# rrahn/libspm

Measured on AMD Instinct MI355X. Metric: Gbases/s scanned, Myers k<=3 |P|=100, higher is better.
Workload: dtype u32

## Files before the change

### libspm_amd/csrc/filter.hpp

```cpp
#pragma once

#include "brute.hpp"
#include "common.hpp"
#include "filter_shared.hpp"
#include "pack.hpp"
#include "hd.hpp"

namespace spm_hip
{

struct survivor
{
    uint32_t key;
    uint32_t t_lo, t_hi;
    uint32_t pad;
};
constexpr uint32_t kSurvInvalid = 0xFFFFFFFFu;

struct band_rec
{
    uint32_t slot;
    uint32_t val;
    uint32_t seg;
    uint32_t band;
// ... 46 lines not shown
        atomicAdd(counter, (unsigned long long)v);
}

__device__ __forceinline__ uint32_t *cand_chunk_of(const filter_params &P, const uint32_t *lds)
{
    const uint32_t wave = (uint32_t)__builtin_amdgcn_readfirstlane(threadIdx.x >> 6);
    return const_cast<uint32_t *>(lds) + P.lds_words + kCandLdsSlot + kCandRec * wave;
}

__device__ __forceinline__ void span_open(const filter_params &P, const uint32_t *lds, uint32_t lane, uint64_t begin)
{
    if (lane == 0) {
        uint32_t *ck = cand_chunk_of(P, lds);
        ck[4] = 0;
        ck[5] = 0;
        ck[6] = (uint32_t)begin;
        ck[7] = (uint32_t)(begin >> 32);
    }
}

__device__ __forceinline__ void span_give_up(const filter_params &P, uint32_t *ck, uint32_t lane)
{
    if (lane == 0) {
        ck[5] = 1;
        const unsigned long long i = atomicAdd(&P.counters[6], 1ull);
        if (i < P.ovf_cap) {
            P.ovf_spans[2 * i] = ((uint64_t)ck[7] << 32) | ck[6];
            P.ovf_spans[2 * i + 1] = (uint64_t)P.span_chunks * (uint64_t)P.span_unit;
        } else {
            atomicAdd(&P.counters[2], 1ull);
        }
    }
    __builtin_amdgcn_fence(__ATOMIC_RELEASE, "wavefront");
    __builtin_amdgcn_wave_barrier();
}

__device__ __forceinline__ void surv_close(const filter_params &P, const uint32_t *ck, uint32_t lane)
{
    const uint32_t used = ck[2], size = ck[3];
    const uint64_t base = ((uint64_t)ck[1] << 32) | ck[0];
    for (uint32_t i = used + lane; i < size; i += 64)
        if (base + i < P.surv_cap) {
            survivor sv;
            sv.key = 0;
            sv.t_lo = 0;
            sv.t_hi = kSurvInvalid;
            sv.pad = 0;
            P.surv[base + i] = sv;
        }
}

__device__ __forceinline__ void emit_survivors(const filter_params &P, bool has, uint32_t key, uint64_t t, uint32_t lane,
                                               const uint32_t *lds)
{
    const uint64_t m = __ballot(has);
    if (m == 0)
        return;
    uint32_t *ck = cand_chunk_of(P, lds);
    const uint32_t n = __popcll(m);
    uint32_t used = (uint32_t)__builtin_amdgcn_readfirstlane(ck[2]);
    const uint32_t size = (uint32_t)__builtin_amdgcn_readfirstlane(ck[3]);
    const uint32_t cnt = (uint32_t)__builtin_amdgcn_readfirstlane(ck[4]) + n;
    if (cnt > P.span_budget) {
        span_give_up(P, ck, lane);
        return;
    }
    if (used + n > size) {
        surv_close(P, ck, lane);
        uint32_t next = size * 2 < kChunkMin ? kChunkMin : (size * 2 > kChunkMax ? kChunkMax : size * 2);
        next = next < n ? n : next;
        if (lane == 0) {
            const unsigned long long b = atomicAdd(&P.counters[1], (unsigned long long)next);
            ck[0] = (uint32_t)b;
            ck[1] = (uint32_t)(b >> 32);
            ck[2] = 0;
            ck[3] = next;
        }
        used = 0;
        __builtin_amdgcn_fence(__ATOMIC_RELEASE, "wavefront");
        __builtin_amdgcn_wave_barrier();
    }
    const uint64_t cbase = ((uint64_t)(uint32_t)__builtin_amdgcn_readfirstlane(ck[1]) << 32) |
                           (uint32_t)__builtin_amdgcn_readfirstlane(ck[0]);
    if (cbase + used + n > P.surv_cap) {
        span_give_up(P, ck, lane);
        return;
    }
    if (has) {
        survivor sv;
        sv.key = key;
        sv.t_lo = (uint32_t)t;
        sv.t_hi = (uint32_t)(t >> 32);
        sv.pad = P.pass;
        P.surv[cbase + used + __popcll(m & ((1ull << lane) - 1))] = sv;
    }
    if (lane == 0) {
        ck[2] = used + n;
        ck[4] = cnt;
    }
    __builtin_amdgcn_fence(__ATOMIC_RELEASE, "wavefront");
    __builtin_amdgcn_wave_barrier();
}

template <int S, int NWD, int HV, int SIG, bool PK, bool KM>
__device__ __forceinline__ void filter_words(const filter_params &P, const uint32_t (&w)[NWD],
                                             const uint32_t (&prev)[NWD], const uint32_t (&nv)[SIG != 4 ? NWD : 1],
                                             uint64_t gbase, uint32_t lane, const uint32_t *lds, uint32_t idx_mask)
{
    constexpr int NWIN = 16 / S;
    const uint32_t kmask = KM ? P.key_mask : 0xFFFFFFFFu;
    static_assert(NWD * NWIN <= 32, "one mask bit per window of a group");
    uint32_t pos_mask = 0;
    if constexpr (HV == 2) {
        const uint16_t *fp_tab = reinterpret_cast<const uint16_t *>(lds);
        const uint16_t *disp_tab = reinterpret_cast<const uint16_t *>(reinterpret_cast<const uint8_t *>(lds) + P.chd_disp_off);
        uint32_t xs[NWD * NWIN], ds[NWD * NWIN];
#pragma unroll
        for (int u = 0; u < NWD; ++u) {
#pragma unroll
            for (int i = 0; i < NWIN; ++i) {
                const int d = S * (i + 1);
                const uint32_t key = (d == 16 ? w[u] : alignbit(w[u], prev[u], (2 * d) & 31)) & kmask;
                const uint32_t x = chd_hash(key).x;
                xs[u * NWIN + i] = x;
                ds[u * NWIN + i] = disp_tab[x >> P.chd_bucket_shift];
            }
        }
#pragma unroll
        for (int u = 0; u < NWD; ++u) {
#pragma unroll
            for (int i = 0; i < NWIN; ++i) {
                const int d = S * (i + 1);
                const uint32_t key = (d == 16 ? w[u] : alignbit(w[u], prev[u], (2 * d) & 31)) & kmask;
                const uint32_t slot = ((xs[u * NWIN + i] >> 3) + ds[u * NWIN + i] * ((key | 1u) & 0xFFFFFFu)) &
                                      P.chd_slot_mask;
                ds[u * NWIN + i] = fp_tab[slot];
            }
        }
#pragma unroll
        for (int u = 0; u < NWD; ++u) {
#pragma unroll
            for (int i = 0; i < NWIN; ++i) {
                const int d = S * (i + 1);
                const uint32_t key = (d == 16 ? w[u] : alignbit(w[u], prev[u], (2 * d) & 31)) & kmask;
                const uint32_t miss = (ds[u * NWIN + i] ^ key ^ (key >> 16)) & 0xFFFFu;
                pos_mask |= (miss == 0 ? 1u : 0u) << (u * NWIN + i);
            }
        }
    } else {
#pragma unroll
        for (int u = 0; u < NWD; ++u) {
#pragma unroll
            for (int i = 0; i < NWIN; ++i) {
                const int d = S * (i + 1);
                const uint32_t key = (d == 16 ? w[u] : alignbit(w[u], prev[u], (2 * d) & 31)) & kmask;
                const uint32_t h = bloom_hash(key, 0) & idx_mask;
                const uint32_t word = lds[h >> 5];
                pos_mask |= __builtin_amdgcn_ubfe(word, h, 1) << (u * NWIN + i);
            }
        }
        for (uint32_t pr = 1; pr < P.n_probes; ++pr) {
            if (__ballot(pos_mask != 0) == 0)
                break;
            uint32_t keep = 0;
#pragma unroll
            for (int u = 0; u < NWD; ++u) {
#pragma unroll
                for (int i = 0; i < NWIN; ++i) {
                    if (pos_mask & (1u << (u * NWIN + i))) {
                        const int d = S * (i + 1);
                        const uint32_t key = (d == 16 ? w[u] : alignbit(w[u], prev[u], (2 * d) & 31)) & kmask;
                        const uint32_t h = bloom_hash(key, pr) & idx_mask;
                        const uint32_t word = lds[h >> 5];
                        keep |= __builtin_amdgcn_ubfe(word, h, 1) << (u * NWIN + i);
                    }
                }
            }
            pos_mask = keep;
        }
    }
    if constexpr (SIG != 4) {
        if (__ballot(pos_mask != 0) != 0) {
#pragma unroll
            for (int u = 0; u < NWD; ++u) {
#pragma unroll
                for (int i = 0; i < NWIN; ++i) {
                    const int d = S * (i + 1);
                    if (__builtin_amdgcn_ubfe(nv[u], d, P.key_len) != 0)
                        pos_mask &= ~(1u << (u * NWIN + i));
                }
            }
        }
    }
    while (__ballot(pos_mask != 0) != 0) {
        if (__builtin_amdgcn_readfirstlane(cand_chunk_of(P, lds)[5]) != 0)
            break;
        uint64_t t = 0;
        uint32_t key = 0;
        bool has = false;
        if (pos_mask != 0) {
            const int bit = __ffs(pos_mask) - 1;
            pos_mask &= pos_mask - 1;
            const int u = bit / NWIN, i = bit % NWIN;
            const int d = S * (i + 1);
            uint32_t wu = w[0], pu = prev[0];
#pragma unroll
            for (int q = 1; q < NWD; ++q)
                if (u == q) {
                    wu = w[q];
                    pu = prev[q];
                }
            key = (d == 16 ? wu : alignbit(wu, pu, (uint32_t)(2 * d) & 31u)) & kmask;
            const uint64_t wpos = PK ? gbase + (uint64_t)(u >> 2) * 4096 + (uint64_t)lane * 64 + (uint64_t)(u & 3) * 16
                                     : gbase + (uint64_t)u * 1024 + (uint64_t)lane * 16;
            const int64_t ts = (int64_t)wpos - 16 + d;
            if (ts >= (int64_t)P.lo && (uint64_t)ts + P.key_len <= P.hi) {
                t = (uint64_t)ts;
                has = true;
            }
        }
        emit_survivors(P, has, key, t, lane, lds);
    }
}



__device__ __forceinline__ uint32_t anchor_select(uint32_t w, uint32_t prev, uint32_t c, uint32_t cm)
{
    const uint32_t C0 = (c & 3u) * 0x55555555u, M0 = (cm & 3u) * 0x55555555u;
    const uint32_t C1 = (c >> 2) * 0x55555555u, M1 = (cm >> 2) * 0x55555555u;
    const uint32_t X = alignbit(w, prev, 2);
    const uint32_t Y = alignbit(w, prev, 4);
    uint32_t t = ((X ^ C0) & M0) | ((Y ^ C1) & M1);
    t |= t >> 1;
    return ~t & 0x55555555u;
}

template <int NWD>
__device__ __forceinline__ void filter_words_anchored(const filter_params &P, const uint32_t (&w)[NWD], const uint32_t (&prev)[NWD],
                                                      uint64_t gbase, uint32_t lane, const uint32_t *lds)
{
    static_assert(NWD % 2 == 0 || NWD == 1, "words are taken in pairs");
    const uint16_t *fp_tab = reinterpret_cast<const uint16_t *>(lds);
    const uint16_t *disp_tab = reinterpret_cast<const uint16_t *>(reinterpret_cast<const uint8_t *>(lds) + P.chd_disp_off);
#pragma unroll
    for (int j = 0; j < NWD; j += 2) {
        uint32_t todo = anchor_select(w[j], prev[j], P.anchor_c, P.anchor_cm);
        if (j + 1 < NWD)
            todo |= anchor_select(w[j + 1 < NWD ? j + 1 : j], prev[j + 1 < NWD ? j + 1 : j], P.anchor_c, P.anchor_cm) << 1;
        while (__ballot(todo != 0) != 0) {
            const bool act = todo != 0;
            const uint32_t b = act ? (uint32_t)__ffs(todo) - 1u : 0u;
            todo &= todo - 1;
            const uint32_t u = b & 1u, d = (b >> 1) + 1u;
            const uint32_t wu = (j + 1 < NWD && u) ? w[j + 1 < NWD ? j + 1 : j] : w[j];
            const uint32_t pu = (j + 1 < NWD && u) ? prev[j + 1 < NWD ? j + 1 : j] : prev[j];
            const uint32_t key = (uint32_t)((((uint64_t)wu << 32) | pu) >> (2 * d));
            const uint32_t x = chd_hash(key).x;
            const uint32_t dsp = disp_tab[x >> P.chd_bucket_shift];
            const uint32_t slot = ((x >> 3) + dsp * ((key | 1u) & 0xFFFFFFu)) & P.chd_slot_mask;
            const uint32_t f = fp_tab[slot];
            const bool hit = act && ((f ^ key ^ (key >> 16)) & 0xFFFFu) == 0;
            if (__ballot(hit) != 0) {
                if (__builtin_amdgcn_readfirstlane(cand_chunk_of(P, lds)[5]) != 0)
                    return;
                const uint64_t wpos = gbase + (uint64_t)(j + u) * 1024 + (uint64_t)lane * 16;
                const int64_t ts = (int64_t)wpos - 16 + (int64_t)d;
                const bool has = hit && ts >= (int64_t)P.lo && (uint64_t)ts + P.key_len <= P.hi;
                emit_survivors(P, has, key, has ? (uint64_t)ts : 0, lane, lds);
            }
        }
    }
}

template <int S, int UU, int HV, int SIG, bool KM, bool AN = false>
__device__ __forceinline__ void filter_group(const filter_params &P, const uint4 (&cur)[UU], uint64_t gbase,
                                             uint32_t &carry_in, uint32_t &carry_n, uint32_t lane,
                                             const uint32_t *lds, uint32_t idx_mask)
{
    uint32_t w[UU], prev[UU];
    uint32_t nv[SIG != 4 ? UU : 1];
#pragma unroll
    for (int u = 0; u < UU; ++u) {
        uint32_t nm = 0;
        w[u] = pack16_sig<SIG>(cur[u], nm);
        prev[u] = __builtin_amdgcn_update_dpp(0u, w[u], 0x138 , 0xF, 0xF, false);
        if (lane == 0)
            prev[u] = carry_in;
        carry_in = __builtin_amdgcn_readlane(w[u], 63);
        if (SIG != 4) {
            uint32_t np = __builtin_amdgcn_update_dpp(0u, nm, 0x138, 0xF, 0xF, false);
            if (lane == 0)
                np = carry_n;
            carry_n = __builtin_amdgcn_readlane(nm, 63);
            nv[u] = (nm << 16) | np;
        }
    }
    if constexpr (AN)
        filter_words_anchored<UU>(P, w, prev, gbase, lane, lds);
    else
        filter_words<S, UU, HV, SIG, false, KM>(P, w, prev, nv, gbase, lane, lds, idx_mask);
}

template <int S, int U, int HV, int SIG, bool KM, bool AN = false>
__global__ __launch_bounds__(((S == 1 && !KM && SIG == 4) || (S == 2 && U == 2)) ? 1024 : 512) void seed_filter_kernel(const filter_params P)
{
    extern __shared__ uint32_t lds[];
    for (uint32_t i = threadIdx.x; i < P.lds_words; i += blockDim.x)
        lds[i] = P.bitmap[i];
    if ((threadIdx.x & 63) == 0) {
        uint32_t *ck = lds + P.lds_words + kCandLdsSlot + kCandRec * (threadIdx.x >> 6);
        for (uint32_t i = 0; i < kCandRec; ++i)
            ck[i] = 0;
    }
    __syncthreads();

    const uint32_t lane = threadIdx.x & 63;
    const uint32_t waves_per_wg = blockDim.x >> 6;
    const uint64_t wave_id =
        (uint64_t)blockIdx.x * waves_per_wg + (uint32_t)__builtin_amdgcn_readfirstlane(threadIdx.x >> 6);
    const uint64_t n_waves = (uint64_t)gridDim.x * waves_per_wg;
    const uint32_t idx_mask = P.bitmap_words * 32 - 1;

    const uint64_t base0 = P.lo & ~1023ull;
    const uint64_t n_chunks = (P.hi - base0 + 1023) / 1024;
    const uint64_t n_whole = (P.hi - base0) / 1024;
    const uint64_t span = P.span_chunks;
    const uint64_t n_spans = (n_chunks + span - 1) / span;
    const uint8_t *lane_text = P.text + base0 + (uint64_t)lane * 16;

    const uint32_t wave_in_wg = (uint32_t)__builtin_amdgcn_readfirstlane(threadIdx.x >> 6);
    uint64_t sp = wave_id;
    for (;;) {
        if (P.dynamic == 1) {
            unsigned long long t = 0;
            if (lane == 0)
                t = atomicAdd(&P.counters[4], 1ull);
            sp = ((unsigned long long)__builtin_amdgcn_readfirstlane((uint32_t)(t >> 32)) << 32) |
                 (uint32_t)__builtin_amdgcn_readfirstlane((uint32_t)t);
        } else if (P.dynamic == 2) {
            __syncthreads();
            if (threadIdx.x == 0) {
                const unsigned long long t = atomicAdd(&P.counters[4], (unsigned long long)waves_per_wg);
                lds[P.lds_words] = (uint32_t)t;
                lds[P.lds_words + 1] = (uint32_t)(t >> 32);
            }
            __syncthreads();
            const uint64_t base = ((uint64_t)(uint32_t)__builtin_amdgcn_readfirstlane(lds[P.lds_words + 1]) << 32) |
                                  (uint32_t)__builtin_amdgcn_readfirstlane(lds[P.lds_words]);
            if (base >= n_spans)
                break;
            sp = base + wave_in_wg;
            if (sp >= n_spans)
                continue;
        }
        if (sp >= n_spans)
            break;
        const uint64_t c_begin = sp * span;
        const uint64_t c_end = c_begin + span < n_chunks ? c_begin + span : n_chunks;
        span_open(P, lds, lane, base0 + c_begin * 1024);
        uint32_t carry_in = 0, carry_n = 0;
        {
            const uint64_t cb = base0 + c_begin * 1024;
            if (cb >= 16 && lane == 0) {
                const uint4 before = load_text16(P.text, cb - 16, P.hi);
                carry_in = pack16_sig<SIG>(before, carry_n);
            }
            carry_in = __builtin_amdgcn_readfirstlane(carry_in);
            carry_n = __builtin_amdgcn_readfirstlane(carry_n);
        }
        uint64_t ch = c_begin;
        const uint64_t whole_end = c_end < n_whole ? c_end : n_whole;
        const uint64_t fast_end = c_begin + (whole_end > c_begin ? (whole_end - c_begin) / U * U : 0);
        if (ch < fast_end) {
            uint4 nxt[U];
#pragma unroll
            for (int u = 0; u < U; ++u)
                nxt[u] = load16_stream(lane_text + (ch + u) * 1024);
            for (; ch < fast_end; ch += U) {
                uint4 cur[U];
#pragma unroll
                for (int u = 0; u < U; ++u)
                    cur[u] = nxt[u];
                const bool more = ch + U < fast_end;
                const uint64_t pf = more ? ch + U : ch;
                const uint64_t ustride = more ? 1024 : 0;
#pragma unroll
                for (int u = 0; u < U; ++u)
                    nxt[u] = load16_stream(lane_text + pf * 1024 + (uint64_t)u * ustride);
                if constexpr (S <= 2)
                    __builtin_amdgcn_sched_barrier(0);
                filter_group<S, U, HV, SIG, KM, AN>(P, cur, base0 + ch * 1024, carry_in, carry_n, lane, lds, idx_mask);
            }
        }
        for (; ch < c_end; ++ch) {
            uint4 one[1];
            one[0] = load_text16(P.text, base0 + ch * 1024 + (uint64_t)lane * 16, P.hi);
            filter_group<S, 1, HV, SIG, KM, AN>(P, one, base0 + ch * 1024, carry_in, carry_n, lane, lds, idx_mask);
        }
        sp += n_waves;
    }
    surv_close(P, cand_chunk_of(P, lds), lane);
}

constexpr uint32_t kDenseQueueCap = 192;
constexpr int kDenseBatches = 3;

template <int NP>
__device__ __forceinline__ uint32_t dense_select(const filter_params &P, uint32_t w, uint32_t prev)
{
    const uint32_t X = alignbit(w, prev, 2);
    const uint32_t Y = alignbit(w, prev, 4);
    uint32_t sel = 0;
#pragma unroll
    for (int i = 0; i < NP; ++i) {
        const uint32_t C0 = (P.pat_c[i] & 3u) * 0x55555555u, M0 = (P.pat_cm[i] & 3u) * 0x55555555u;
        const uint32_t C1 = (P.pat_c[i] >> 2) * 0x55555555u, M1 = (P.pat_cm[i] >> 2) * 0x55555555u;
        uint32_t t = ((X ^ C0) & M0) | ((Y ^ C1) & M1);
        t |= t >> 1;
        sel |= ~t;
    }
    return sel & 0x55555555u;
}

struct dense_queue
{
    uint32_t key[kDenseQueueCap];
    uint32_t off[kDenseQueueCap];
};

__device__ __forceinline__ void dense_drain(const filter_params &P, dense_queue &Q, uint32_t &qn, bool all, uint64_t span_base,
                                            uint32_t lane, const uint32_t *lds)
{
    while (qn >= 64 || (all && qn != 0)) {
        const uint32_t nb_full = qn >> 6;
        uint32_t nb = all ? (qn + 63) >> 6 : nb_full;
        nb = nb > (uint32_t)kDenseBatches ? (uint32_t)kDenseBatches : nb;
        uint32_t key[kDenseBatches], off[kDenseBatches];
        uint4 bk[kDenseBatches];
        bool v[kDenseBatches];
#pragma unroll
        for (int b = 0; b < kDenseBatches; ++b) {
            const int32_t e = (int32_t)qn - 64 * b - 1 - (int32_t)lane;
            v[b] = (uint32_t)b < nb && e >= 0;
            key[b] = 0;
            off[b] = 0;
            bk[b] = make_uint4(0, 0, 0, 0);
            if (v[b]) {
                key[b] = Q.key[e];
                off[b] = Q.off[e];
                bk[b] = P.buckets[dense_bucket(key[b], P.bucket_shift)];
            }
        }
        qn = qn > 64 * nb ? qn - 64 * nb : 0;
#pragma unroll
        for (int b = 0; b < kDenseBatches; ++b) {
            if ((uint32_t)b >= nb)
                break;
            const uint32_t f2 = dense_fp(key[b]) * 0x00010001u;
            const uint32_t x0 = bk[b].x ^ f2, x1 = bk[b].y ^ f2, x2 = bk[b].z ^ f2, x3 = bk[b].w ^ f2;
            const uint32_t z = ((x0 - 0x00010001u) & ~x0) | ((x1 - 0x00010001u) & ~x1) | ((x2 - 0x00010001u) & ~x2) |
                               ((x3 - 0x00010001u) & ~x3);
            const bool hit = v[b] && ((z & 0x80008000u) != 0 || (bk[b].w >> 16) == kDenseAcceptAll);
            if (__ballot(hit) != 0) {
                if (__builtin_amdgcn_readfirstlane(cand_chunk_of(P, lds)[5]) == 0) {
                    const int64_t ts = (int64_t)span_base + (int64_t)off[b] - 16;
                    const bool has = hit && ts >= (int64_t)P.lo && (uint64_t)ts + P.key_len <= P.hi;
                    emit_survivors(P, has, key[b], has ? (uint64_t)ts : 0, lane, lds);
                }
            }
        }
    }
}

template <int UU, int NP, int S, bool KM>
__device__ __forceinline__ void dense_group(const filter_params &P, const uint4 (&cur)[UU], uint64_t gbase, uint64_t span_base,
                                            uint32_t &carry_in, uint32_t lane, const uint32_t *lds, dense_queue &Q, uint32_t &qn)
{
    static_assert(UU % 2 == 0 || UU == 1, "words are taken in pairs");
    uint32_t w[UU], prev[UU];
#pragma unroll
    for (int u = 0; u < UU; ++u) {
        w[u] = pack16(cur[u]);
        prev[u] = __builtin_amdgcn_update_dpp(0u, w[u], 0x138 , 0xF, 0xF, false);
        if (lane == 0)
            prev[u] = carry_in;
        carry_in = __builtin_amdgcn_readlane(w[u], 63);
    }
    const uint32_t goff = (uint32_t)(gbase - span_base) + lane * 16;
#pragma unroll
    for (int j = 0; j < UU; j += 2) {
        constexpr bool pair = UU > 1;
        const uint32_t w0 = w[j], p0 = prev[j], w1 = w[pair ? j + 1 : j], p1 = prev[pair ? j + 1 : j];
        const uint32_t kmask = KM ? P.key_mask : 0xFFFFFFFFu;
        static_assert(kDenseBloomBits == 20, "the word address below takes bits 5..19 of the index");
        uint32_t pm = 0;
        if constexpr (S == 0) {
            uint32_t todo = dense_select<NP>(P, w0, p0);
            if (pair)
                todo |= dense_select<NP>(P, w1, p1) << 1;
            while (todo != 0) {
                const uint32_t b = (uint32_t)__ffs(todo) - 1u;
                todo &= todo - 1;
                const bool odd = (b & 1u) != 0;
                const uint64_t both = ((uint64_t)(odd ? w1 : w0) << 32) | (odd ? p1 : p0);
                const uint32_t key = (uint32_t)(both >> ((b & ~1u) + 2u));
                const uint32_t h = key ^ (key >> 13);
                const uint32_t word = *reinterpret_cast<const uint32_t *>(reinterpret_cast<const uint8_t *>(lds) + ((h >> 3) & 0x1FFFCu));
                pm |= __builtin_amdgcn_ubfe(word, h, 1) << b;
            }
        } else {
#pragma unroll
            for (int u = 0; u < (pair ? 2 : 1); ++u) {
#pragma unroll
                for (int d = S; d <= 16; d += S) {
                    const uint32_t wu = u ? w1 : w0, pu = u ? p1 : p0;
                    const uint32_t key = (d == 16 ? wu : alignbit(wu, pu, (2 * d) & 31)) & kmask;
                    const uint32_t h = key ^ (key >> 13);
                    const uint32_t word = *reinterpret_cast<const uint32_t *>(reinterpret_cast<const uint8_t *>(lds) + ((h >> 3) & 0x1FFFCu));
                    pm |= __builtin_amdgcn_ubfe(word, h, 1) << (2 * (d - 1) + u);
                }
            }
        }
        while (__ballot(pm != 0) != 0) {
            const bool pos = pm != 0;
            const uint32_t b = pos ? (uint32_t)__ffs(pm) - 1u : 0u;
            pm &= pm - 1;
            const bool odd = (b & 1u) != 0;
            const uint64_t both = ((uint64_t)(odd ? w1 : w0) << 32) | (odd ? p1 : p0);
            const uint32_t key = (uint32_t)(both >> ((b & ~1u) + 2u)) & kmask;
            const uint64_t mm = __ballot(pos);
            if (pos) {
                const uint32_t q = qn + __popcll(mm & ((1ull << lane) - 1));
                Q.key[q] = key;
                Q.off[q] = goff + (uint32_t)j * 1024u + (odd ? 1024u : 0u) + (b >> 1) + 1u;
            }
            qn += __popcll(mm);
            __builtin_amdgcn_fence(__ATOMIC_RELEASE, "wavefront");
            __builtin_amdgcn_wave_barrier();
            if (qn > kDenseQueueCap - 64)
                dense_drain(P, Q, qn, false, span_base, lane, lds);
        }
    }
}

template <int U, int NP, int S = 0, bool KM = false>
__global__ __launch_bounds__(1024) void seed_filter_dense_kernel(const filter_params P)
{
    extern __shared__ uint32_t lds[];
    for (uint32_t i = threadIdx.x; i < P.lds_words; i += blockDim.x)
        lds[i] = P.bitmap[i];
    if ((threadIdx.x & 63) == 0) {
        uint32_t *ck = lds + P.lds_words + kCandLdsSlot + kCandRec * (threadIdx.x >> 6);
        for (uint32_t i = 0; i < kCandRec; ++i)
            ck[i] = 0;
    }
    __syncthreads();

    const uint32_t lane = threadIdx.x & 63;
    const uint32_t waves_per_wg = blockDim.x >> 6;
    const uint32_t wave_in_wg = (uint32_t)__builtin_amdgcn_readfirstlane(threadIdx.x >> 6);
    const uint64_t wave_id = (uint64_t)blockIdx.x * waves_per_wg + wave_in_wg;
    const uint64_t n_waves = (uint64_t)gridDim.x * waves_per_wg;
    dense_queue &Q = *reinterpret_cast<dense_queue *>(lds + P.lds_words + kCandLdsSlot + kCandRec * 16 +
                                                      (sizeof(dense_queue) / 4) * wave_in_wg);
    uint32_t qn = 0;

    const uint64_t base0 = P.lo & ~1023ull;
    const uint64_t n_chunks = (P.hi - base0 + 1023) / 1024;
    const uint64_t n_whole = (P.hi - base0) / 1024;
    const uint64_t span = P.span_chunks;
    const uint64_t n_spans = (n_chunks + span - 1) / span;
    const uint8_t *lane_text = P.text + base0 + (uint64_t)lane * 16;

    uint64_t sp = wave_id;
    for (;;) {
        if (P.dynamic == 1) {
            unsigned long long t = 0;
            if (lane == 0)
                t = atomicAdd(&P.counters[4], 1ull);
            sp = ((unsigned long long)__builtin_amdgcn_readfirstlane((uint32_t)(t >> 32)) << 32) |
                 (uint32_t)__builtin_amdgcn_readfirstlane((uint32_t)t);
        } else if (P.dynamic == 2) {
            __syncthreads();
            if (threadIdx.x == 0) {
                const unsigned long long t = atomicAdd(&P.counters[4], (unsigned long long)waves_per_wg);
                lds[P.lds_words] = (uint32_t)t;
                lds[P.lds_words + 1] = (uint32_t)(t >> 32);
            }
            __syncthreads();
            const uint64_t base = ((uint64_t)(uint32_t)__builtin_amdgcn_readfirstlane(lds[P.lds_words + 1]) << 32) |
                                  (uint32_t)__builtin_amdgcn_readfirstlane(lds[P.lds_words]);
            if (base >= n_spans)
                break;
            sp = base + wave_in_wg;
            if (sp >= n_spans)
                continue;
        }
        if (sp >= n_spans)
            break;
        const uint64_t c_begin = sp * span;
        const uint64_t c_end = c_begin + span < n_chunks ? c_begin + span : n_chunks;
        const uint64_t span_base = base0 + c_begin * 1024;
        span_open(P, lds, lane, span_base);
        uint32_t carry_in = 0;
        {
            uint32_t nm = 0;
            if (span_base >= 16 && lane == 0)
                carry_in = pack16_sig<4>(load_text16(P.text, span_base - 16, P.hi), nm);
            carry_in = __builtin_amdgcn_readfirstlane(carry_in);
        }
        uint64_t ch = c_begin;
        const uint64_t whole_end = c_end < n_whole ? c_end : n_whole;
        const uint64_t fast_end = c_begin + (whole_end > c_begin ? (whole_end - c_begin) / U * U : 0);
        if (ch < fast_end) {
            uint4 nxt[U];
#pragma unroll
            for (int u = 0; u < U; ++u)
                nxt[u] = load16_stream(lane_text + (ch + u) * 1024);
            for (; ch < fast_end; ch += U) {
                uint4 cur[U];
#pragma unroll
                for (int u = 0; u < U; ++u)
                    cur[u] = nxt[u];
                const bool more = ch + U < fast_end;
                const uint64_t pf = more ? ch + U : ch;
                const uint64_t ustride = more ? 1024 : 0;
#pragma unroll
                for (int u = 0; u < U; ++u)
                    nxt[u] = load16_stream(lane_text + pf * 1024 + (uint64_t)u * ustride);
                __builtin_amdgcn_sched_barrier(0);
                dense_group<U, NP, S, KM>(P, cur, base0 + ch * 1024, span_base, carry_in, lane, lds, Q, qn);
            }
        }
        for (; ch < c_end; ++ch) {
            uint4 one[1];
            one[0] = load_text16(P.text, base0 + ch * 1024 + (uint64_t)lane * 16, P.hi);
            dense_group<1, NP, S, KM>(P, one, base0 + ch * 1024, span_base, carry_in, lane, lds, Q, qn);
        }
        dense_drain(P, Q, qn, true, span_base, lane, lds);
        sp += n_waves;
    }
    surv_close(P, cand_chunk_of(P, lds), lane);
}

template <int S, int U2, int HV, bool KM>
__global__ __launch_bounds__(1024) void seed_filter_packed_kernel(const filter_params P, const uint4 *__restrict__ shadow)
{
    extern __shared__ uint32_t lds[];
    for (uint32_t i = threadIdx.x; i < P.lds_words; i += blockDim.x)
        lds[i] = P.bitmap[i];
    if ((threadIdx.x & 63) == 0) {
        uint32_t *ck = lds + P.lds_words + kCandLdsSlot + kCandRec * (threadIdx.x >> 6);
        for (uint32_t i = 0; i < kCandRec; ++i)
            ck[i] = 0;
    }
    __syncthreads();

    constexpr int NWD = 4 * U2;
    const uint32_t lane = threadIdx.x & 63;
    const uint32_t waves_per_wg = blockDim.x >> 6;
    const uint32_t wave_in_wg = (uint32_t)__builtin_amdgcn_readfirstlane(threadIdx.x >> 6);
    const uint64_t wave_id = (uint64_t)blockIdx.x * waves_per_wg + wave_in_wg;
    const uint64_t n_waves = (uint64_t)gridDim.x * waves_per_wg;
    const uint32_t idx_mask = P.bitmap_words * 32 - 1;

    const uint64_t base0 = P.lo & ~4095ull;
    const uint64_t n_chunks = (P.hi - base0 + 4095) / 4096;
    const uint64_t span = P.span_chunks;
    const uint64_t n_spans = (n_chunks + span - 1) / span;
    const uint4 *lane_src = shadow + (base0 / 64) + lane;

    uint64_t sp = wave_id;
    for (;;) {
        if (P.dynamic == 1) {
            unsigned long long t = 0;
            if (lane == 0)
                t = atomicAdd(&P.counters[4], 1ull);
            sp = ((unsigned long long)__builtin_amdgcn_readfirstlane((uint32_t)(t >> 32)) << 32) |
                 (uint32_t)__builtin_amdgcn_readfirstlane((uint32_t)t);
        } else if (P.dynamic == 2) {
            __syncthreads();
            if (threadIdx.x == 0) {
                const unsigned long long t = atomicAdd(&P.counters[4], (unsigned long long)waves_per_wg);
                lds[P.lds_words] = (uint32_t)t;
                lds[P.lds_words + 1] = (uint32_t)(t >> 32);
            }
            __syncthreads();
            const uint64_t base = ((uint64_t)(uint32_t)__builtin_amdgcn_readfirstlane(lds[P.lds_words + 1]) << 32) |
                                  (uint32_t)__builtin_amdgcn_readfirstlane(lds[P.lds_words]);
            if (base >= n_spans)
                break;
            sp = base + wave_in_wg;
            if (sp >= n_spans)
                continue;
        }
        if (sp >= n_spans)
            break;
        const uint64_t c_begin = sp * span;
        const uint64_t c_end = c_begin + span < n_chunks ? c_begin + span : n_chunks;
        const uint64_t fast_end = c_begin + (c_end - c_begin + U2 - 1) / U2 * U2;
        span_open(P, lds, lane, base0 + c_begin * 4096);
        uint32_t carry_in = 0;
        {
            const uint64_t first_word = (base0 + c_begin * 4096) / 16;
            if (first_word > 0 && lane == 0)
                carry_in = reinterpret_cast<const uint32_t *>(shadow)[first_word - 1];
            carry_in = __builtin_amdgcn_readfirstlane(carry_in);
        }
        uint4 nxt[U2];
#pragma unroll
        for (int u = 0; u < U2; ++u)
            nxt[u] = load16_stream(reinterpret_cast<const uint8_t *>(lane_src + (c_begin + u) * 64));
        for (uint64_t ch = c_begin; ch < fast_end; ch += U2) {
            uint4 cur[U2];
#pragma unroll
            for (int u = 0; u < U2; ++u)
                cur[u] = nxt[u];
            const bool more = ch + U2 < fast_end;
            const uint64_t pf = more ? ch + U2 : ch;
            const uint64_t ustride = more ? 64 : 0;
#pragma unroll
            for (int u = 0; u < U2; ++u)
                nxt[u] = load16_stream(reinterpret_cast<const uint8_t *>(lane_src + pf * 64 + (uint64_t)u * ustride));
            __builtin_amdgcn_sched_barrier(0);
            uint32_t w[NWD], prev[NWD];
            const uint32_t nv[1] = {0};
#pragma unroll
            for (int u = 0; u < U2; ++u) {
                w[4 * u + 0] = cur[u].x;
                w[4 * u + 1] = cur[u].y;
                w[4 * u + 2] = cur[u].z;
                w[4 * u + 3] = cur[u].w;
                uint32_t p0 = __builtin_amdgcn_update_dpp(0u, cur[u].w, 0x138 , 0xF, 0xF, false);
                if (lane == 0)
                    p0 = carry_in;
                carry_in = __builtin_amdgcn_readlane(cur[u].w, 63);
                prev[4 * u + 0] = p0;
                prev[4 * u + 1] = cur[u].x;
                prev[4 * u + 2] = cur[u].y;
                prev[4 * u + 3] = cur[u].z;
            }
            filter_words<S, NWD, HV, 4, true, KM>(P, w, prev, nv, base0 + ch * 4096, lane, lds, idx_mask);
        }
        sp += n_waves;
    }
    surv_close(P, cand_chunk_of(P, lds), lane);
}

struct verify_params
{
    const uint8_t *text;
    uint64_t text_alloc;
    uint64_t ctx_begin;
    uint64_t scan_begin;
    uint64_t scan_end;
    uint64_t pos_offset;
    const band_rec *bands;
    const unsigned long long *counters;
    uint32_t band_counter;
    uint32_t preselected;
    uint64_t band_cap;
    ulonglong2 *band_tab;
    uint32_t table_mask, band_bits;
    uint32_t runs;
    const uint8_t *surplus;
    uint32_t Bw;
    uint32_t overlap;
    uint32_t max_m;
    const uint32_t *peq32;
    uint32_t sigma;
    uint32_t nw_table;
    uint32_t max_k;
    const int32_t *m;
    const int32_t *k;
    uint32_t report_begin;
    uint32_t max_span;
    uint32_t wave_text;
    unsigned long long *seen;
    uint32_t seen_mask;
    spm_hit *hits;
    unsigned long long *hit_counter;
    uint64_t hit_cap;
    unsigned long long *overflow;
    const uint64_t *seg_offsets;
    uint64_t n_segments;
    const uint32_t *seg_owned;
};

struct resolve_params
{
    const survivor *surv;
    unsigned long long *counters;
    uint64_t surv_cap;
    const pass_entry *passes;
    const uint4 *entries;
    uint32_t key_len;
    uint32_t flank_check;
    uint32_t pieces_check;
    const uint8_t *text;
    uint64_t text_alloc;
    const uint8_t *needle_ranks;
    const uint32_t *needle_offsets;
    const uint16_t *seed_q;
    const int32_t *m, *k;
    uint64_t hay_begin, hay_end;
    const uint64_t *seg_offsets;
    uint64_t n_segments;
    uint32_t Bw, overlap, max_m;
    uint32_t band_bits;
    ulonglong2 *band_tab;
    uint32_t table_mask;
    band_rec *bands;
    uint64_t band_cap;
    const uint32_t *needle_pk;
    const uint32_t *pk_offsets;
    uint32_t exact_hits;
    uint32_t report_begin;
    uint64_t scan_begin, scan_end;
    uint64_t pos_offset;
    const uint32_t *seg_owned;
    unsigned long long *seen;
    uint32_t seen_mask;
    spm_hit *hits;
    unsigned long long *hit_counter, *overflow;
    uint64_t hit_cap;
    uint32_t *table_poison;
};

__device__ __forceinline__ unsigned long long band_value(unsigned long long stored, bool counting)
{
    return counting ? (unsigned long long)(uint32_t)(stored + 1ull) : ~stored;
}
__device__ __forceinline__ void band_release(ulonglong2 *tab, uint32_t slot)
{
    tab[slot] = make_ulonglong2(kBandEmpty, ~0ull);
}

__device__ __forceinline__ uint4 load_bytes16(const uint8_t *p)
{
    uint4 v;
    __builtin_memcpy(&v, p, 16);
    return v;
}

__device__ __forceinline__ uint4 load_bytes16_guarded(const uint8_t *base, uint64_t idx, uint64_t limit)
{
    if (idx + 16 <= limit)
        return load_bytes16(base + idx);
    uint32_t w[4] = {0xFFFFFFFFu, 0xFFFFFFFFu, 0xFFFFFFFFu, 0xFFFFFFFFu};
    for (int b = 0; b < 16; ++b)
        if (idx + b < limit)
            w[b >> 2] = (w[b >> 2] & ~(0xFFu << (8 * (b & 3)))) | ((uint32_t)base[idx + b] << (8 * (b & 3)));
    return make_uint4(w[0], w[1], w[2], w[3]);
}

__device__ __forceinline__ uint32_t diff16(const uint4 a, const uint4 b, uint32_t n)
{
    const uint32_t d[4] = {a.x ^ b.x, a.y ^ b.y, a.z ^ b.z, a.w ^ b.w};
    uint32_t r = 0;
#pragma unroll
    for (uint32_t i = 0; i < 4; ++i) {
        const uint32_t have = n > 4 * i ? n - 4 * i : 0;
        const uint32_t mask = have >= 4 ? 0xFFFFFFFFu : (have == 0 ? 0u : (1u << (8 * have)) - 1);
        r |= d[i] & mask;
    }
    return r;
}

__device__ __forceinline__ bool seed_intact(const resolve_params &P, uint64_t t, uint32_t val, uint32_t r, uint32_t q_whole,
                                            int64_t hay_b, int64_t hay_e)
{
    if (!P.needle_ranks)
        return true;
    const uint32_t pat = val >> 11, x = val & 0x7FF;
    struct
    {
        uint32_t q;
    } sp{q_whole ? q_whole : P.seed_q[pat]};
    const uint32_t o = x - r;
    const int64_t ts = (int64_t)t - (int64_t)r;
    if (ts < hay_b || ts + (int64_t)sp.q > hay_e)
        return false;
    const uint8_t *nd = P.needle_ranks + P.needle_offsets[pat] + o;
    for (uint32_t i = 0; i < sp.q; i += 16) {
        const uint32_t n = sp.q - i < 16 ? sp.q - i : 16;
        if (diff16(load_bytes16_guarded(P.text, (uint64_t)ts + i, P.text_alloc), load_bytes16(nd + i), n))
            return false;
    }
    return true;
}

constexpr uint32_t kPieceRoundsShift = 21, kPieceMissingShift = 28;

__device__ __forceinline__ bool pieces_apply(const resolve_params &P, uint64_t t, uint32_t val, uint32_t m, uint32_t k, int64_t hay_b,
                                             int64_t hay_e)
{
    if (!P.pieces_check || k == 0 || k > 7 || m < 32)
        return false;
    const int64_t d = (int64_t)t - (int64_t)(val & 0x7FF);
    return d - (int64_t)k >= hay_b && d + (int64_t)(m + k) <= hay_e;
}

__device__ __forceinline__ uint32_t pieces_visit(const resolve_params &P, uint64_t t, uint32_t val, uint32_t &rng, uint32_t m, uint32_t k)
{
    const uint32_t pat = val >> 11, x = val & 0x7FF;
    const uint32_t n_rounds = m >> 4;
    uint32_t done = (rng >> kPieceRoundsShift) & 0x7F, missing = (rng >> kPieceMissingShift) & 7;
    const bool ascending = 2 * x >= m;
    const uint32_t todo = n_rounds - done < 2 ? n_rounds - done : 2;
    const uint32_t r_lo = ascending ? done : n_rounds - done - todo;
    const uint32_t *pk = P.needle_pk + P.pk_offsets[pat] + r_lo;
    const uint32_t nw0 = pk[0], nw1 = todo == 2 ? pk[1] : 0;
    const uint64_t w0 = (uint64_t)((int64_t)t - (int64_t)x + (int64_t)(16 * r_lo) - (int64_t)k);
    const uint32_t c0 = pack16(load_bytes16_guarded(P.text, w0, P.text_alloc));
    const uint32_t c1 = pack16(load_bytes16_guarded(P.text, w0 + 16, P.text_alloc));
    const uint32_t c2 = todo == 2 ? pack16(load_bytes16_guarded(P.text, w0 + 32, P.text_alloc)) : 0;
#pragma unroll
    for (uint32_t rr = 0; rr < 2; ++rr) {
        if (rr < todo) {
            const uint32_t two = rr ? nw1 : nw0;
            const uint64_t win = rr ? ((uint64_t)c1 | ((uint64_t)c2 << 32)) : ((uint64_t)c0 | ((uint64_t)c1 << 32));
#pragma unroll
            for (uint32_t j = 0; j < 2; ++j) {
                const uint32_t piece = (two >> (16 * j)) & 0xFFFFu;
                bool found = false;
                for (uint32_t sh = 0; sh <= 2 * k; ++sh)
                    found = found || (((uint32_t)(win >> (2 * (8 * j + sh))) & 0xFFFFu) == piece);
                missing += found ? 0u : 1u;
            }
        }
    }
    if (missing > k)
        return 0;
    done += todo;
    if (done >= n_rounds)
        return 2;
    rng = (rng & ~((0x7Fu << kPieceRoundsShift) | (7u << kPieceMissingShift))) | (done << kPieceRoundsShift) |
          (missing << kPieceMissingShift);
    return 1;
}

struct text64
{
    uint64_t lo, hi;
    bool ok;
};

__device__ __forceinline__ uint32_t syms16(const text64 &W, uint32_t first)
{
    if (first >= 32)
        return (uint32_t)(W.hi >> (2 * (first - 32)));
    return (uint32_t)(W.lo >> (2 * first)) | (first ? (uint32_t)(W.hi << (2 * (32 - first)) ) : 0u);
}
// ... 1098 lines not shown
```

Baseline: 6422.

## Vectorize LDS table staging and prefetch first span text before staging

Replaces the scalar per-word copy of the bitmap table into LDS with batched 16-byte loads, eight in flight per thread, shared by the three filter kernels. In seed_filter_kernel, span scheduling moves into span_first/span_next helpers, and each span's first text chunks plus the 16-byte carry word are issued before the table copy and barrier, so the loads overlap the staging. This is meant to hide kernel prologue and per-span start latency, at the cost of more live registers and a restructured dynamic-scheduling loop. The dynamic==1 path now adds n_waves to the atomic counter value, which changes which span each wave takes first.

Result: faster. 6517, median of 6 (+1.5%).

```diff
diff --git a/libspm_amd/csrc/filter.hpp b/libspm_amd/csrc/filter.hpp
--- a/libspm_amd/csrc/filter.hpp
+++ b/libspm_amd/csrc/filter.hpp
@@ -372,18 +372,78 @@
         filter_words<S, UU, HV, SIG, false, KM>(P, w, prev, nv, gbase, lane, lds, idx_mask);
 }
 
+constexpr int kStageLoads = 8;
+
+__device__ __forceinline__ void stage_table(const filter_params &P, uint32_t *lds)
+{
+    const uint32_t n4 = P.lds_words >> 2;
+    const uint4 *src = reinterpret_cast<const uint4 *>(P.bitmap);
+    uint4 *dst = reinterpret_cast<uint4 *>(lds);
+    for (uint32_t i0 = threadIdx.x; i0 < n4; i0 += kStageLoads * blockDim.x) {
+        uint4 v[kStageLoads];
+#pragma unroll
+        for (int b = 0; b < kStageLoads; ++b) {
+            const uint32_t i = i0 + b * blockDim.x;
+            v[b] = src[i < n4 ? i : n4 - 1];
+        }
+#pragma unroll
+        for (int b = 0; b < kStageLoads; ++b) {
+            const uint32_t i = i0 + b * blockDim.x;
+            dst[i < n4 ? i : n4 - 1] = v[b];
+        }
+    }
+    for (uint32_t i = 4 * n4 + threadIdx.x; i < P.lds_words; i += blockDim.x)
+        lds[i] = P.bitmap[i];
+}
+
+constexpr uint32_t kSpanDone = 0, kSpanIdle = 1, kSpanWork = 2;
+
+__device__ __forceinline__ uint32_t span_first(const filter_params &P, uint64_t n_spans, uint64_t wave_id)
+{
+    if (P.dynamic == 2 && (uint64_t)blockIdx.x * (blockDim.x >> 6) >= n_spans)
+        return kSpanDone;
+    return wave_id < n_spans ? kSpanWork : (P.dynamic == 2 ? kSpanIdle : kSpanDone);
+}
+
+__device__ __forceinline__ uint32_t span_next(const filter_params &P, uint32_t *lds, uint32_t lane, uint64_t n_spans,
+                                              uint64_t n_waves, uint64_t &sp)
+{
+    if (P.dynamic == 1) {
+        unsigned long long t = 0;
+        if (lane == 0)
+            t = atomicAdd(&P.counters[4], 1ull);
+        sp = n_waves + (((unsigned long long)__builtin_amdgcn_readfirstlane((uint32_t)(t >> 32)) << 32) |
+                        (uint32_t)__builtin_amdgcn_readfirstlane((uint32_t)t));
+    } else if (P.dynamic == 2) {
+        __syncthreads();
+        if (threadIdx.x == 0) {
+            const unsigned long long t = atomicAdd(&P.counters[4], (unsigned long long)(blockDim.x >> 6));
+            lds[P.lds_words] = (uint32_t)t;
+            lds[P.lds_words + 1] = (uint32_t)(t >> 32);
+        }
+        __syncthreads();
+        const uint64_t base = n_waves + (((uint64_t)(uint32_t)__builtin_amdgcn_readfirstlane(lds[P.lds_words + 1]) << 32) |
+                                         (uint32_t)__builtin_amdgcn_readfirstlane(lds[P.lds_words]));
+        if (base >= n_spans)
+            return kSpanDone;
+        sp = base + (uint32_t)__builtin_amdgcn_readfirstlane(threadIdx.x >> 6);
+        if (sp >= n_spans)
+            return kSpanIdle;
+    } else {
+        sp += n_waves;
+    }
+    return sp < n_spans ? kSpanWork : kSpanDone;
+}
+
 template <int S, int U, int HV, int SIG, bool KM, bool AN = false>
 __global__ __launch_bounds__(((S == 1 && !KM && SIG == 4) || (S == 2 && U == 2)) ? 1024 : 512) void seed_filter_kernel(const filter_params P)
 {
     extern __shared__ uint32_t lds[];
-    for (uint32_t i = threadIdx.x; i < P.lds_words; i += blockDim.x)
-        lds[i] = P.bitmap[i];
     if ((threadIdx.x & 63) == 0) {
         uint32_t *ck = lds + P.lds_words + kCandLdsSlot + kCandRec * (threadIdx.x >> 6);
         for (uint32_t i = 0; i < kCandRec; ++i)
             ck[i] = 0;
     }
-    __syncthreads();
 
     const uint32_t lane = threadIdx.x & 63;
     const uint32_t waves_per_wg = blockDim.x >> 6;
@@ -399,43 +459,37 @@
     const uint64_t n_spans = (n_chunks + span - 1) / span;
     const uint8_t *lane_text = P.text + base0 + (uint64_t)lane * 16;
 
-    const uint32_t wave_in_wg = (uint32_t)__builtin_amdgcn_readfirstlane(threadIdx.x >> 6);
     uint64_t sp = wave_id;
-    for (;;) {
-        if (P.dynamic == 1) {
-            unsigned long long t = 0;
-            if (lane == 0)
-                t = atomicAdd(&P.counters[4], 1ull);
-            sp = ((unsigned long long)__builtin_amdgcn_readfirstlane((uint32_t)(t >> 32)) << 32) |
-                 (uint32_t)__builtin_amdgcn_readfirstlane((uint32_t)t);
-        } else if (P.dynamic == 2) {
-            __syncthreads();
-            if (threadIdx.x == 0) {
-                const unsigned long long t = atomicAdd(&P.counters[4], (unsigned long long)waves_per_wg);
-                lds[P.lds_words] = (uint32_t)t;
-                lds[P.lds_words + 1] = (uint32_t)(t >> 32);
-            }
-            __syncthreads();
-            const uint64_t base = ((uint64_t)(uint32_t)__builtin_amdgcn_readfirstlane(lds[P.lds_words + 1]) << 32) |
-                                  (uint32_t)__builtin_amdgcn_readfirstlane(lds[P.lds_words]);
-            if (base >= n_spans)
-                break;
-            sp = base + wave_in_wg;
-            if (sp >= n_spans)
-                continue;
-        }
-        if (sp >= n_spans)
-            break;
+    uint32_t st = span_first(P, n_spans, wave_id);
+    uint4 nxt[U], before = make_uint4(0, 0, 0, 0);
+    auto span_loads = [&]() {
+        if (st != kSpanWork)
+            return;
+        const uint64_t c_begin = sp * span;
+        const uint64_t c_end = c_begin + span < n_chunks ? c_begin + span : n_chunks;
+        const uint64_t cb = base0 + c_begin * 1024;
+        if (cb >= 16)
+            before = *reinterpret_cast<const uint4 *>(P.text + cb - 16);
+        if (c_begin + U <= (c_end < n_whole ? c_end : n_whole))
+#pragma unroll
+            for (int u = 0; u < U; ++u)
+                nxt[u] = load16_stream(lane_text + (c_begin + u) * 1024);
+    };
+    span_loads();
+    stage_table(P, lds);
+    __syncthreads();
+
+    for (; st != kSpanDone; st = span_next(P, lds, lane, n_spans, n_waves, sp), span_loads()) {
+        if (st == kSpanIdle)
+            continue;
         const uint64_t c_begin = sp * span;
         const uint64_t c_end = c_begin + span < n_chunks ? c_begin + span : n_chunks;
         span_open(P, lds, lane, base0 + c_begin * 1024);
         uint32_t carry_in = 0, carry_n = 0;
         {
             const uint64_t cb = base0 + c_begin * 1024;
-            if (cb >= 16 && lane == 0) {
-                const uint4 before = load_text16(P.text, cb - 16, P.hi);
+            if (cb >= 16 && lane == 0)
                 carry_in = pack16_sig<SIG>(before, carry_n);
-            }
             carry_in = __builtin_amdgcn_readfirstlane(carry_in);
             carry_n = __builtin_amdgcn_readfirstlane(carry_n);
         }
@@ -443,10 +497,6 @@
         const uint64_t whole_end = c_end < n_whole ? c_end : n_whole;
         const uint64_t fast_end = c_begin + (whole_end > c_begin ? (whole_end - c_begin) / U * U : 0);
         if (ch < fast_end) {
-            uint4 nxt[U];
-#pragma unroll
-            for (int u = 0; u < U; ++u)
-                nxt[u] = load16_stream(lane_text + (ch + u) * 1024);
             for (; ch < fast_end; ch += U) {
                 uint4 cur[U];
 #pragma unroll
@@ -468,7 +518,6 @@
             one[0] = load_text16(P.text, base0 + ch * 1024 + (uint64_t)lane * 16, P.hi);
             filter_group<S, 1, HV, SIG, KM, AN>(P, one, base0 + ch * 1024, carry_in, carry_n, lane, lds, idx_mask);
         }
-        sp += n_waves;
     }
     surv_close(P, cand_chunk_of(P, lds), lane);
 }
@@ -618,8 +667,7 @@
 __global__ __launch_bounds__(1024) void seed_filter_dense_kernel(const filter_params P)
 {
     extern __shared__ uint32_t lds[];
-    for (uint32_t i = threadIdx.x; i < P.lds_words; i += blockDim.x)
-        lds[i] = P.bitmap[i];
+    stage_table(P, lds);
     if ((threadIdx.x & 63) == 0) {
         uint32_t *ck = lds + P.lds_words + kCandLdsSlot + kCandRec * (threadIdx.x >> 6);
         for (uint32_t i = 0; i < kCandRec; ++i)
@@ -718,8 +766,7 @@
 __global__ __launch_bounds__(1024) void seed_filter_packed_kernel(const filter_params P, const uint4 *__restrict__ shadow)
 {
     extern __shared__ uint32_t lds[];
-    for (uint32_t i = threadIdx.x; i < P.lds_words; i += blockDim.x)
-        lds[i] = P.bitmap[i];
+    stage_table(P, lds);
     if ((threadIdx.x & 63) == 0) {
         uint32_t *ck = lds + P.lds_words + kCandLdsSlot + kCandRec * (threadIdx.x >> 6);
         for (uint32_t i = 0; i < kCandRec; ++i)
```
